# juankim834/RecommendSystemProject

Hardware: AMD Instinct MI355X
Metric: training samples/sec (user-item pairs) at batch 4096; 1/2/4/8 MI355X (higher is better)
Workload: dtype bf16; 1 GPU; c2: MovieLens-1M DSSM + Transformer seq encoder (seq_len 50, d=64); global_batch=4096, per_gpu_batch=4096, seq_len=50, dropout=config, parallelism=dp1, hip_graph=True, ids=uniform, hard_negatives=0, resident_batches=8, deterministic=True

## Files before the change

recommendsystemproject_amd/csrc/attention.hip:

```cpp
#include <type_traits>

#include "attn_rows.h"
#include "common.h"
#include "mfma.h"
#include "rng.h"

namespace rs {
namespace {

__device__ __forceinline__ bool map_bh(int B, int H, int& b, int& h) {
  const int bid = blockIdx.x, xcd = bid & 7, slot = bid >> 3;
  b = (slot / H) * 8 + xcd;
  h = slot % H;
  return b < B;
}

__host__ inline int bh_grid(int B, int H) { return ((B + 7) / 8) * 8 * H; }

template <int HD, bool DROP>
__global__ __launch_bounds__(256) void attn_fwd_kernel(const float* __restrict__ qkv,
                                                       const uint8_t* __restrict__ key_pad,
                                                       float* __restrict__ out,
                                                       float* __restrict__ lse, int B, int L,
                                                       int d, int H, float scale, float pdrop,
// ... 228 lines not shown
    for (int tk = 0; tk < NT; ++tk)
#pragma unroll
      for (int s4 = 0; s4 < 4; ++s4) o = mfma4(sv[tk][s4], Vs[tk * 16 + 4 * q + s4][r], o);
    if (q == 0 && i < L) lse[(int64_t)bh * L + i] = (m + log2f(l)) * kLn2;
#pragma unroll
    for (int e = 0; e < 4; ++e) {
      const float le = __shfl(l, 4 * q + e, 64);
      const int row = tq * 16 + 4 * q + e;
      if (row < L) out[((int64_t)b * L + row) * d + h * 16 + r] = o[e] * (1.f / le);
    }
  }
}

template <int NT, bool DROP>
__global__ __launch_bounds__(256) void attn_bwd_mfma_kernel(
    const float* __restrict__ qkv, const uint8_t* __restrict__ key_pad,
    const float* __restrict__ out, const float* __restrict__ dout, const float* __restrict__ lse,
    float* __restrict__ dqkv, int B, int L, int d, int H, float scale, float pdrop,
    const int64_t* __restrict__ key, int site) {
  constexpr int LP = NT * 16;
  constexpr int TP = 20;
  __shared__ __attribute__((aligned(16))) float Qsm[4][LP][kRowP];
  __shared__ __attribute__((aligned(16))) float Ksm[4][LP][kRowP];
  __shared__ __attribute__((aligned(16))) float Gsm[4][LP][kRowP];
  __shared__ __attribute__((aligned(16))) float Tsm[4][LP * TP];
  const int wave = threadIdx.x >> 6, lane = threadIdx.x & 63;
  const int r = lane & 15, q = lane >> 4;
  const int bh = blockIdx.x * 4 + wave;
  if (bh >= B * H) return;
  const int b = bh / H, h = bh % H;
  const int ld = 3 * d;
  const float* base = qkv + (int64_t)b * L * ld + h * 16;
  const float* gbase = dout + (int64_t)b * L * d + h * 16;
  const float* obase = out + (int64_t)b * L * d + h * 16;
  float(*Qs)[kRowP] = Qsm[wave];
  float(*Ks)[kRowP] = Ksm[wave];
  float(*Gs)[kRowP] = Gsm[wave];
  float* T = Tsm[wave];
  f4 qf[NT], kf[NT], vf[NT], gf[NT];
  float Di[NT], lsei[NT];
#pragma unroll
  for (int t = 0; t < NT; ++t) {
    const int row = t * 16 + r;
    const f4 z = {0.f, 0.f, 0.f, 0.f};
    const bool ok = row < L;
    qf[t] = ok ? ld4(base + (int64_t)row * ld + 4 * q) : z;
    kf[t] = ok ? ld4(base + (int64_t)row * ld + d + 4 * q) : z;
    vf[t] = ok ? ld4(base + (int64_t)row * ld + 2 * d + 4 * q) : z;
    gf[t] = ok ? ld4(gbase + (int64_t)row * d + 4 * q) : z;
    const f4 of = ok ? ld4(obase + (int64_t)row * d + 4 * q) : z;
    *reinterpret_cast<f4*>(&Qs[row][4 * q]) = qf[t];
    *reinterpret_cast<f4*>(&Ks[row][4 * q]) = kf[t];
    *reinterpret_cast<f4*>(&Gs[row][4 * q]) = gf[t];
    Di[t] = quad_sum(gf[t][0] * of[0] + gf[t][1] * of[1] + gf[t][2] * of[2] + gf[t][3] * of[3]);
    lsei[t] = ok ? lse[(int64_t)bh * L + row] * kLog2e : 0.f;
  }
  bool kok[NT][4];
#pragma unroll
  for (int t = 0; t < NT; ++t)
#pragma unroll
    for (int e = 0; e < 4; ++e) {
      const int j = t * 16 + 4 * q + e;
      kok[t][e] = j < L && key_pad[(int64_t)b * L + j] == 0;
    }
  DropKey dk;
  if (DROP) dk = make_key(key, site, pdrop);
  const float scale2 = scale * kLog2e;
  __builtin_amdgcn_wave_barrier();
  float* dbase = dqkv + (int64_t)b * L * ld + h * 16;
  f4 dv_acc[NT], dk_acc[NT];
#pragma unroll
  for (int t = 0; t < NT; ++t) dv_acc[t] = dk_acc[t] = f4{0.f, 0.f, 0.f, 0.f};
#pragma unroll
  for (int tq = 0; tq < NT; ++tq) {
    const int i = tq * 16 + r;
    const uint32_t rowbase = ((uint32_t)bh * (uint32_t)L + (uint32_t)i) * (uint32_t)L;
    f4 ps[NT], ds[NT];
#pragma unroll
    for (int tk = 0; tk < NT; ++tk) {
      f4 sacc = {0.f, 0.f, 0.f, 0.f}, pacc = {0.f, 0.f, 0.f, 0.f};
#pragma unroll
      for (int s4 = 0; s4 < 4; ++s4) {
        sacc = mfma4(kf[tk][s4], qf[tq][s4], sacc);
        pacc = mfma4(vf[tk][s4], gf[tq][s4], pacc);
      }
      float mk[4] = {1.f, 1.f, 1.f, 1.f};
      if (DROP) keep4_32(dk, rowbase + tk * 16 + 4 * q, mk);
#pragma unroll
      for (int e = 0; e < 4; ++e) {
        const float pv = (kok[tk][e] && i < L) ? exp2f(sacc[e] * scale2 - lsei[tq]) : 0.f;
        const float z = DROP ? mk[e] : 1.f;
        ds[tk][e] = pv * (z * pacc[e] - Di[tq]);
        ps[tk][e] = pv * z;
      }
    }
    f4 dq = {0.f, 0.f, 0.f, 0.f};
#pragma unroll
    for (int tk = 0; tk < NT; ++tk)
#pragma unroll
      for (int s4 = 0; s4 < 4; ++s4) dq = mfma4(ds[tk][s4], Ks[tk * 16 + 4 * q + s4][r], dq);
#pragma unroll
    for (int e = 0; e < 4; ++e) {
      const int row = tq * 16 + 4 * q + e;
      if (row < L) dbase[(int64_t)row * ld + r] = dq[e] * scale;
    }
#pragma unroll
    for (int tk = 0; tk < NT; ++tk)
#pragma unroll
      for (int e = 0; e < 4; ++e) T[(tk * 16 + 4 * q + e) * TP + r] = ps[tk][e];
    __builtin_amdgcn_wave_barrier();
#pragma unroll
    for (int tk = 0; tk < NT; ++tk) {
      const f4 a = ld4(&T[(tk * 16 + r) * TP + 4 * q]);
#pragma unroll
      for (int s4 = 0; s4 < 4; ++s4) dv_acc[tk] = mfma4(a[s4], Gs[tq * 16 + 4 * q + s4][r], dv_acc[tk]);
    }
    __builtin_amdgcn_wave_barrier();
#pragma unroll
    for (int tk = 0; tk < NT; ++tk)
#pragma unroll
      for (int e = 0; e < 4; ++e) T[(tk * 16 + 4 * q + e) * TP + r] = ds[tk][e];
    __builtin_amdgcn_wave_barrier();
#pragma unroll
    for (int tk = 0; tk < NT; ++tk) {
      const f4 a = ld4(&T[(tk * 16 + r) * TP + 4 * q]);
#pragma unroll
      for (int s4 = 0; s4 < 4; ++s4) dk_acc[tk] = mfma4(a[s4], Qs[tq * 16 + 4 * q + s4][r], dk_acc[tk]);
    }
    __builtin_amdgcn_wave_barrier();
  }
#pragma unroll
  for (int tk = 0; tk < NT; ++tk)
#pragma unroll
    for (int e = 0; e < 4; ++e) {
      const int row = tk * 16 + 4 * q + e;
      if (row < L) {
        dbase[(int64_t)row * ld + d + r] = dk_acc[tk][e] * scale;
        dbase[(int64_t)row * ld + 2 * d + r] = dv_acc[tk][e];
      }
    }
}


__device__ __forceinline__ shortx4 bf4(const f4& v) {
  typedef __bf16 bf2v __attribute__((ext_vector_type(2)));
  typedef float f2v __attribute__((ext_vector_type(2)));
  const bf2v lo = __builtin_convertvector(f2v{v[0], v[1]}, bf2v);
  const bf2v hi = __builtin_convertvector(f2v{v[2], v[3]}, bf2v);
  return __builtin_bit_cast(shortx4, __builtin_shufflevector(lo, hi, 0, 1, 2, 3));
}
__device__ __forceinline__ f4 mfma16(const shortx4& a, const shortx4& b, const f4& c) {
  return __builtin_amdgcn_mfma_f32_16x16x16bf16_1k(a, b, c, 0, 0, 0);
}
template <int NT, int P>
__device__ __forceinline__ void col_frags(const float* X, int r, int q, shortx4 (&out)[NT]) {
#pragma unroll
  for (int t = 0; t < NT; ++t) {
    f4 v;
#pragma unroll
    for (int j = 0; j < 4; ++j) v[j] = X[(t * 16 + 4 * q + j) * P + r];
    out[t] = bf4(v);
  }
}

__device__ __forceinline__ void stq(float* p, float v) { *p = v; }
__device__ __forceinline__ void stq(__bf16* p, float v) { *p = (__bf16)v; }

template <int NT>
__device__ __forceinline__ uint32_t key_bits(const uint8_t* __restrict__ key_pad, int b, int L,
                                             int lane, int q) {
  const bool valid = lane < L && key_pad[(int64_t)b * L + lane] == 0;
  const uint64_t vm = __ballot(valid);
  uint32_t kb = 0;
#pragma unroll
  for (int t = 0; t < NT; ++t) kb |= (uint32_t)((vm >> (16 * t + 4 * q)) & 0xFu) << (4 * t);
  return kb;
}

__device__ __forceinline__ void attn_keep4(const DropKey& dk, bool leven, uint32_t idx0, float (&mk)[4]) {
  if (leven) {
    keep_pair32(dk, idx0 >> 1, mk[0], mk[1]);
    keep_pair32(dk, (idx0 >> 1) + 1, mk[2], mk[3]);
  } else {
    keep4_32(dk, idx0, mk);
  }
}

__device__ __forceinline__ void attn_keep4b(const DropKey& dk, bool leven, uint32_t idx0, bool (&kp)[4]) {
  if (leven) {
    const uint32_t h0 = pair_hash32(dk, idx0 >> 1), h1 = pair_hash32(dk, (idx0 >> 1) + 1);
    kp[0] = (h0 & 0xffffu) >= dk.thresh;
    kp[1] = (h0 >> 16) >= dk.thresh;
    kp[2] = (h1 & 0xffffu) >= dk.thresh;
    kp[3] = (h1 >> 16) >= dk.thresh;
  } else {
#pragma unroll
    for (int i = 0; i < 4; ++i) {
      const uint32_t x = idx0 + i, hh = pair_hash32(dk, x >> 1);
      kp[i] = ((x & 1) ? (hh >> 16) : (hh & 0xffffu)) >= dk.thresh;
    }
  }
}

template <int NT>
__device__ __forceinline__ void key_bias(uint32_t kbits, f4 (&kbias)[NT]) {
#pragma unroll
  for (int t = 0; t < NT; ++t)
#pragma unroll
    for (int e = 0; e < 4; ++e) kbias[t][e] = ((kbits >> (4 * t + e)) & 1u) ? 0.f : -INFINITY;
}
__device__ __forceinline__ float vmax(float a, float b) { return __builtin_elementwise_maximum(a, b); }

__device__ __forceinline__ shortx4 tr_col(const __bf16* W, int wp, int tk, int lane) {
  const int g = lane >> 4, l16 = lane & 15;
  return tr4(W + (4 * g + (l16 >> 2)) * wp + 16 * tk + 4 * (l16 & 3));
}

template <int TP>
__device__ __forceinline__ f4 tile_rows(float* T, const f4& acc, int r, int q, int lane) {
#pragma unroll
  for (int e = 0; e < 4; ++e) T[(4 * q + e) * TP + r] = acc[e];
  __builtin_amdgcn_wave_barrier();
  const f4 v = ld4(&T[(lane >> 2) * TP + 4 * (lane & 3)]);
  __builtin_amdgcn_wave_barrier();
  return v;
}

template <int NT, bool DROP, bool QB, bool ZB = false>
__global__ __launch_bounds__(256) void attn_fwd_bf16_kernel(
    const void* __restrict__ qkv_, const uint8_t* __restrict__ key_pad, float* __restrict__ out,
    float* __restrict__ lse, int B, int L, int d, int H, float scale, float pdrop,
    const int64_t* __restrict__ key, int site, uint16_t* __restrict__ zbits = nullptr) {
  constexpr int LP = NT * 16;
  __shared__ __attribute__((aligned(16))) float Vsm[4][LP][kRowP];
  const int wave = threadIdx.x >> 6, lane = threadIdx.x & 63;
  const int r = lane & 15, q = lane >> 4;
  const int bh = blockIdx.x * 4 + wave;
  if (bh >= B * H) return;
  const int b = bh / H, h = bh % H;
  const int ld = 3 * d;
  typedef typename std::conditional<QB, __bf16, float>::type QT;
  const QT* base = reinterpret_cast<const QT*>(qkv_) + (int64_t)b * L * ld + h * 16;
  float(*Vs)[kRowP] = Vsm[wave];
  shortx4 qb[NT], kb[NT], vb[NT];
#pragma unroll
  for (int t = 0; t < NT; ++t) {
    const int row = t * 16 + r;
    const f4 z = {0.f, 0.f, 0.f, 0.f};
    qb[t] = bf4(row < L ? ld4(base + (int64_t)row * ld + 4 * q) : z);
    kb[t] = bf4(row < L ? ld4(base + (int64_t)row * ld + d + 4 * q) : z);
    *reinterpret_cast<f4*>(&Vs[row][4 * q]) = row < L ? ld4(base + (int64_t)row * ld + 2 * d + 4 * q) : z;
  }
  const uint32_t kbits = key_bits<NT>(key_pad, b, L, lane, q);
  f4 kbias[NT];
  key_bias<NT>(kbits, kbias);
  DropKey dk;
  if (DROP) dk = make_key(key, site, pdrop);
  const bool leven = (L & 1) == 0;
  const float scale2 = scale * kLog2e;
  __builtin_amdgcn_wave_barrier();
  col_frags<NT, kRowP>(&Vs[0][0], r, q, vb);
  __builtin_amdgcn_wave_barrier();
  float* T = &Vs[0][0];
#pragma unroll
  for (int tq = 0; tq < NT; ++tq) {
    f4 sv[NT];
#pragma unroll
    for (int tk = 0; tk < NT; ++tk) sv[tk] = mfma16(kb[tk], qb[tq], kbias[tk]);
    float m = -INFINITY;
#pragma unroll
    for (int tk = 0; tk < NT; ++tk) m = vmax(vmax(vmax(m, sv[tk][0]), sv[tk][1]), vmax(sv[tk][2], sv[tk][3]));
    m = quad_max(m);
    const float ms = m == -INFINITY ? 0.f : m * scale2;
    float l = 0.f;
    const int i = tq * 16 + r;
    const uint32_t rowbase = ((uint32_t)bh * (uint32_t)L + (uint32_t)i) * (uint32_t)L;
    uint32_t zw = 0;
#pragma unroll
    for (int tk = 0; tk < NT; ++tk) {
      bool kp[4] = {true, true, true, true};
      if (DROP) attn_keep4b(dk, leven, rowbase + tk * 16 + 4 * q, kp);
#pragma unroll
      for (int e = 0; e < 4; ++e) {
        const float pv = __builtin_amdgcn_exp2f(__builtin_fmaf(sv[tk][e], scale2, -ms));
        l += pv;
        sv[tk][e] = kp[e] ? pv : 0.f;
        if (ZB) zw |= kp[e] ? (1u << (4 * tk + e)) : 0u;
      }
    }
    if (ZB) zbits[((int64_t)bh * NT + tq) * 64 + lane] = (uint16_t)zw;
    l = quad_sum(l);
    f4 o = {0.f, 0.f, 0.f, 0.f};
#pragma unroll
    for (int tk = 0; tk < NT; ++tk) o = mfma16(bf4(sv[tk]), vb[tk], o);
    if (q == 0 && i < L) lse[(int64_t)bh * L + i] = (ms + __builtin_amdgcn_logf(l)) * kLn2;
    const float rl = DROP ? __builtin_amdgcn_rcpf(l) * dk.scale : __builtin_amdgcn_rcpf(l);
    f4 on;
#pragma unroll
    for (int e = 0; e < 4; ++e) on[e] = o[e] * __shfl(rl, 4 * q + e, 64);
    const f4 v = tile_rows<kRowP>(T, on, r, q, lane);
    const int row = tq * 16 + (lane >> 2);
    if (row < L) put4(out + ((int64_t)b * L + row) * d + h * 16 + 4 * (lane & 3), v);
  }
}

template <int NT, bool DROP, bool QB, bool ZB = false>
__global__ __launch_bounds__(256, 3) void attn_bwd_bf16_kernel(
    const void* __restrict__ qkv_, const uint8_t* __restrict__ key_pad,
    const float* __restrict__ out, const float* __restrict__ dout, const float* __restrict__ lse,
    void* __restrict__ dqkv_, int B, int L, int d, int H, float scale, float pdrop,
    const int64_t* __restrict__ key, int site, const uint16_t* __restrict__ zbits = nullptr) {
  constexpr int LP = NT * 16;
  constexpr int TP = 24;
  constexpr int WP = LP + 16;
  constexpr int XW = (LP * TP > 16 * TP + 16 * WP) ? LP * TP : 16 * TP + 16 * WP;
  __shared__ __attribute__((aligned(16))) float Xsm[4][XW];
  __shared__ __attribute__((aligned(16))) shortx4 Fsm[4][2][NT][64];
  const int wave = threadIdx.x >> 6, lane = threadIdx.x & 63;
  const int r = lane & 15, q = lane >> 4;
  const int bh = blockIdx.x * 4 + wave;
  if (bh >= B * H) return;
  const int b = bh / H, h = bh % H;
  const int ld = 3 * d;
  typedef typename std::conditional<QB, __bf16, float>::type QT;
  const QT* base = reinterpret_cast<const QT*>(qkv_) + (int64_t)b * L * ld + h * 16;
  const float* gbase = dout + (int64_t)b * L * d + h * 16;
  float* T = Xsm[wave];
  shortx4 qb[NT], kb[NT], vb[NT], gb[NT];
  float lsei[NT];
  shortx4 kc[NT];
  {
    f4 qf[NT], kf[NT], gf[NT];
#pragma unroll
    for (int t = 0; t < NT; ++t) {
      const int row = t * 16 + r;
      const f4 z = {0.f, 0.f, 0.f, 0.f};
      const bool ok = row < L;
      qf[t] = ok ? ld4(base + (int64_t)row * ld + 4 * q) : z;
      kf[t] = ok ? ld4(base + (int64_t)row * ld + d + 4 * q) : z;
      vb[t] = bf4(ok ? ld4(base + (int64_t)row * ld + 2 * d + 4 * q) : z);
      gf[t] = ok ? ld4(gbase + (int64_t)row * d + 4 * q) : z;
      const float ls = ok ? lse[(int64_t)bh * L + row] : 0.f;
      lsei[t] = !ok ? INFINITY : (ls == -INFINITY ? 0.f : ls * kLog2e);
    }
#pragma unroll
    for (int pass = 0; pass < 3; ++pass) {
#pragma unroll
      for (int t = 0; t < NT; ++t)
        *reinterpret_cast<f4*>(&T[(t * 16 + r) * TP + 4 * q]) = pass == 0 ? qf[t] : (pass == 1 ? kf[t] : gf[t]);
      __builtin_amdgcn_wave_barrier();
      if (pass == 1) {
        col_frags<NT, TP>(T, r, q, kc);
      } else {
        shortx4 cf[NT];
        col_frags<NT, TP>(T, r, q, cf);
#pragma unroll
        for (int t = 0; t < NT; ++t) Fsm[wave][pass >> 1][t][lane] = cf[t];
      }
      __builtin_amdgcn_wave_barrier();
    }
#pragma unroll
    for (int t = 0; t < NT; ++t) {
      qb[t] = bf4(qf[t]);
      kb[t] = bf4(kf[t]);
      gb[t] = bf4(gf[t]);
    }
  }
  uint32_t zw[NT];
  if (ZB)
#pragma unroll
    for (int t = 0; t < NT; ++t) zw[t] = zbits[((int64_t)bh * NT + t) * 64 + lane];
  const uint32_t kbits = key_bits<NT>(key_pad, b, L, lane, q);
  f4 kbias[NT];
  key_bias<NT>(kbits, kbias);
  DropKey dk;
  if (DROP) dk = make_key(key, site, pdrop);
  const bool leven = (L & 1) == 0;
  const float scale2 = scale * kLog2e;
  const float zs = DROP ? dk.scale : 1.f;
  QT* dbase = reinterpret_cast<QT*>(dqkv_) + (int64_t)b * L * ld + h * 16;
  __bf16* Wpz = reinterpret_cast<__bf16*>(T + 16 * TP);
  __bf16* Wds = Wpz + 16 * WP;
  f4 dv_acc[NT], dk_acc[NT];
#pragma unroll
  for (int t = 0; t < NT; ++t) dv_acc[t] = dk_acc[t] = f4{0.f, 0.f, 0.f, 0.f};
#pragma unroll
  for (int tq = 0; tq < NT; ++tq) {
    const int i = tq * 16 + r;
    const uint32_t rowbase = ((uint32_t)bh * (uint32_t)L + (uint32_t)i) * (uint32_t)L;
    f4 pvs[NT], dpz[NT];
    float Dp = 0.f;
#pragma unroll
    for (int tk = 0; tk < NT; ++tk) {
      const f4 sacc = mfma16(kb[tk], qb[tq], kbias[tk]);
      const f4 pacc = mfma16(vb[tk], gb[tq], f4{0.f, 0.f, 0.f, 0.f});
      bool kp[4] = {true, true, true, true};
      if (ZB) {
#pragma unroll
        for (int e = 0; e < 4; ++e) kp[e] = (zw[tq] >> (4 * tk + e)) & 1u;
      } else if (DROP) {
        attn_keep4b(dk, leven, rowbase + tk * 16 + 4 * q, kp);
      }
      f4 pz;
#pragma unroll
      for (int e = 0; e < 4; ++e) {
        const float pv = __builtin_amdgcn_exp2f(__builtin_fmaf(sacc[e], scale2, -lsei[tq]));
        pvs[tk][e] = pv;
        dpz[tk][e] = kp[e] ? pacc[e] : 0.f;
        pz[e] = kp[e] ? pv : 0.f;
        Dp = __builtin_fmaf(pv, dpz[tk][e], Dp);
      }
      *reinterpret_cast<shortx4*>(&Wpz[r * WP + 16 * tk + 4 * q]) = bf4(pz);
    }
    const float Di = quad_sum(Dp) * zs;
    f4 dq = {0.f, 0.f, 0.f, 0.f};
#pragma unroll
    for (int tk = 0; tk < NT; ++tk) {
      f4 ds;
#pragma unroll
      for (int e = 0; e < 4; ++e) ds[e] = pvs[tk][e] * __builtin_fmaf(dpz[tk][e], zs, -Di);
      const shortx4 dsb = bf4(ds);
      *reinterpret_cast<shortx4*>(&Wds[r * WP + 16 * tk + 4 * q]) = dsb;
      dq = mfma16(dsb, kc[tk], dq);
    }
    __builtin_amdgcn_wave_barrier();
#pragma unroll
    for (int tk = 0; tk < NT; ++tk) {
      dv_acc[tk] = mfma16(tr_col(Wpz, WP, tk, lane), Fsm[wave][1][tq][lane], dv_acc[tk]);
      dk_acc[tk] = mfma16(tr_col(Wds, WP, tk, lane), Fsm[wave][0][tq][lane], dk_acc[tk]);
    }
    {
      const f4 v = tile_rows<TP>(T, dq * scale, r, q, lane);
      const int row = tq * 16 + (lane >> 2);
      if (row < L) put4(dbase + (int64_t)row * ld + 4 * (lane & 3), v);
    }
    __builtin_amdgcn_wave_barrier();
  }
#pragma unroll
  for (int tk = 0; tk < NT; ++tk) {
    const f4 vk = tile_rows<TP>(T, dk_acc[tk] * scale, r, q, lane);
    const f4 vv = tile_rows<TP>(T, dv_acc[tk] * zs, r, q, lane);
    const int row = tk * 16 + (lane >> 2);
    if (row < L) {
      put4(dbase + (int64_t)row * ld + d + 4 * (lane & 3), vk);
      put4(dbase + (int64_t)row * ld + 2 * d + 4 * (lane & 3), vv);
    }
  }
}

template <int NT>
__device__ __forceinline__ uint64_t key_bits_long(const uint8_t* __restrict__ key_pad, int b,
                                                  int L, int lane, int q) {
  uint64_t kb = 0;
#pragma unroll
  for (int g = 0; g < (NT + 3) / 4; ++g) {
    const int j = 64 * g + lane;
    const uint64_t vm = __ballot(j < L && key_pad[(int64_t)b * L + j] == 0);
#pragma unroll
    for (int tt = 0; tt < 4; ++tt)
      if (4 * g + tt < NT) kb |= ((vm >> (16 * tt + 4 * q)) & 0xFull) << (4 * (4 * g + tt));
  }
  return kb;
}

template <int LP, typename QT>
__device__ __forceinline__ void load_head_image(const QT* __restrict__ base, int ld, int L,
                                                int off, float (*X)[kRowP]) {
  for (int e = threadIdx.x; e < LP * 4; e += 256) {
    const int row = e >> 2, c4 = (e & 3) * 4;
    f4 v = {0.f, 0.f, 0.f, 0.f};
    if (row < L) v = ld4(base + (int64_t)row * ld + off + c4);
    *reinterpret_cast<f4*>(&X[row][c4]) = v;
  }
}

__device__ __forceinline__ void keep_col4(const DropKey& dk, bool leven, uint32_t rb0, uint32_t L,
                                          uint32_t j, int r, float (&mk)[4]) {
  if (leven) {
    const int p = r & 1;
    float mine[2], recv[2];
#pragma unroll
    for (int s = 0; s < 2; ++s) {
      const uint32_t e = 2 * p + s;
      const uint32_t h = pair_hash32(dk, (rb0 + e * L + (j & ~1u)) >> 1);
      const float lo = (h & 0xffffu) >= dk.thresh ? dk.scale : 0.f;
      const float hi = (h >> 16) >= dk.thresh ? dk.scale : 0.f;
      mine[s] = p ? hi : lo;
      recv[s] = __shfl_xor(p ? lo : hi, 1, 64);
    }
#pragma unroll
    for (int e = 0; e < 4; ++e) mk[e] = ((e >> 1) == p) ? mine[e & 1] : recv[e & 1];
  } else {
#pragma unroll
    for (int e = 0; e < 4; ++e) mk[e] = keep_mult32(dk, rb0 + e * L + j);
  }
}

constexpr int kRowPB = 24;
template <int LP, typename QT>
__device__ __forceinline__ void load_head_image16(const QT* __restrict__ base, int ld, int L, int off,
                                                  __bf16 (*X)[kRowPB]) {
  for (int e = threadIdx.x; e < LP * 4; e += 256) {
    const int row = e >> 2, c4 = (e & 3) * 4;
    f4 v = {0.f, 0.f, 0.f, 0.f};
    if (row < L) v = ld4(base + (int64_t)row * ld + off + c4);
    *reinterpret_cast<shortx4*>(&X[row][c4]) = bf4(v);
  }
}
__device__ __forceinline__ shortx4 row_frag16(const __bf16 (*X)[kRowPB], int row, int q) {
  return *reinterpret_cast<const shortx4*>(&X[row][4 * q]);
}
__device__ __forceinline__ shortx4 col_frag16(const __bf16 (*X)[kRowPB], int t0, int r, int q) {
  shortx4 o;
#pragma unroll
  for (int j = 0; j < 4; ++j) o[j] = __builtin_bit_cast(short, X[t0 + 4 * q + j][r]);
  return o;
}

#ifndef RS_LONG_FWD_MINW
#define RS_LONG_FWD_MINW 3
#endif
template <int NT, bool DROP, bool QB>
__global__ __launch_bounds__(256, RS_LONG_FWD_MINW) void attn_fwd_long_bf16_kernel(
    const void* __restrict__ qkv_, const uint8_t* __restrict__ key_pad, float* __restrict__ out,
    float* __restrict__ lse, int B, int L, int d, int H, float scale, float pdrop,
    const int64_t* __restrict__ key, int site) {
  constexpr int LP = NT * 16;
  __shared__ __attribute__((aligned(16))) __bf16 Qs[LP][kRowPB];
  __shared__ __attribute__((aligned(16))) __bf16 Ks[LP][kRowPB];
  __shared__ __attribute__((aligned(16))) __bf16 Vs[LP][kRowPB];
  __shared__ __attribute__((aligned(16))) float Tsm[4][16 * kRowP];
  __shared__ __attribute__((aligned(16))) float Kb[LP];
  int b, h;
  if (!map_bh(B, H, b, h)) return;
  const int bh = b * H + h;
  const int wave = threadIdx.x >> 6, lane = threadIdx.x & 63;
  const int r = lane & 15, q = lane >> 4;
  const int ld = 3 * d;
  typedef typename std::conditional<QB, __bf16, float>::type QT;
  const QT* base = reinterpret_cast<const QT*>(qkv_) + (int64_t)b * L * ld + h * 16;
  load_head_image16<LP>(base, ld, L, 0, Qs);
  load_head_image16<LP>(base, ld, L, d, Ks);
  load_head_image16<LP>(base, ld, L, 2 * d, Vs);
  for (int j = threadIdx.x; j < LP; j += 256) Kb[j] = (j < L && key_pad[(int64_t)b * L + j] == 0) ? 0.f : -INFINITY;
  DropKey dk;
  if (DROP) dk = make_key(key, site, pdrop);
  const bool leven = (L & 1) == 0;
  const float scale2 = scale * kLog2e;
  __syncthreads();
  shortx4 kb[NT];
#pragma unroll
  for (int t = 0; t < NT; ++t) kb[t] = row_frag16(Ks, t * 16 + r, q);
  float* T = Tsm[wave];
  constexpr int NTF = 4 * (NT / 4), NR = NT - NTF;
  for (int tq = wave; tq < NTF; tq += 4) {
    const int i = tq * 16 + r;
    const f4 z = {0.f, 0.f, 0.f, 0.f};
    const shortx4 qb = row_frag16(Qs, i, q);
    constexpr int CH = 4;
    float m = -INFINITY, ms = 0.f, l = 0.f;
    f4 o = z;
    const uint32_t rowbase = ((uint32_t)bh * (uint32_t)L + (uint32_t)i) * (uint32_t)L;
#pragma unroll
    for (int c0 = 0; c0 < NT; c0 += CH) {
      f4 sv[CH];
      float cm = -INFINITY;
#pragma unroll
      for (int u = 0; u < CH; ++u) {
        const int tk = c0 + u;
        if (tk >= NT) break;
        sv[u] = mfma16(kb[tk], qb, ld4(&Kb[tk * 16 + 4 * q]));
        cm = vmax(vmax(vmax(cm, sv[u][0]), sv[u][1]), vmax(sv[u][2], sv[u][3]));
      }
      cm = quad_max(cm);
      const float mn = vmax(m, cm);
      const float msn = mn == -INFINITY ? 0.f : mn * scale2;
      if (c0 > 0) {
        const float al = m == -INFINITY ? 0.f : __builtin_amdgcn_exp2f(ms - msn);
        l *= al;
#pragma unroll
        for (int e = 0; e < 4; ++e) o[e] *= __shfl(al, 4 * q + e, 64);
      }
      m = mn;
      ms = msn;
#pragma unroll
      for (int u = 0; u < CH; ++u) {
        const int tk = c0 + u;
        if (tk >= NT) break;
        bool kp[4] = {true, true, true, true};
        if (DROP) attn_keep4b(dk, leven, rowbase + tk * 16 + 4 * q, kp);
#pragma unroll
        for (int e = 0; e < 4; ++e) {
          const float pv = __builtin_amdgcn_exp2f(__builtin_fmaf(sv[u][e], scale2, -ms));
          l += pv;
// ... 151 lines not shown
    L2s[i] = li;
    Kv[i] = kv;
  }
  DropKey dk;
  if (DROP) dk = make_key(key, site, pdrop);
  const bool leven = (L & 1) == 0;
  const float scale2 = scale * kLog2e;
  const f4 z = {0.f, 0.f, 0.f, 0.f};
  float* T = reinterpret_cast<float*>(Tbs[wave]);
  __bf16* Tb = Tbs[wave];
  QT* dbase = reinterpret_cast<QT*>(dqkv_) + (int64_t)b * L * ld + h * 16;
  __syncthreads();

  shortx4 kr[NW], vr[NW], kc[NW];
  float kval[NW];
  f4 dk_acc[NW], dv_acc[NW], dq_acc[NT];
#pragma unroll
  for (int u = 0; u < NW; ++u) {
    const int tk = u < NW0 ? wave + 4 * u : NTF + (u - NW0);
    kr[u] = row_frag16(Ks, tk * 16 + r, q);
    vr[u] = row_frag16(Vs, tk * 16 + r, q);
    kc[u] = col_frag16(Ks, tk * 16, r, q);
    kval[u] = Kv[tk * 16 + r];
    dk_acc[u] = dv_acc[u] = z;
  }
#pragma unroll
  for (int tq = 0; tq < NT; ++tq) {
    const shortx4 qr = row_frag16(Qs, tq * 16 + r, q);
    const shortx4 gr = row_frag16(Gs, tq * 16 + r, q);
    const shortx4 qc[1] = {col_frag16(Qs, tq * 16, r, q)};
    const shortx4 gc[1] = {col_frag16(Gs, tq * 16, r, q)};
    const f4 l2 = ld4(&L2s[tq * 16 + 4 * q]);
    const f4 Dq = ld4(&Ds[tq * 16 + 4 * q]);
    dq_acc[tq] = z;
#pragma unroll
    for (int u = 0; u < NW; ++u) {
      const int tk = u < NW0 ? wave + 4 * u : NTF + (u - NW0);
      if (u >= NW0 && (tq & 3) != wave) continue;
      const f4 sacc = mfma16(qr, kr[u], z);
      const f4 pacc = mfma16(gr, vr[u], z);
      float mk[4] = {1.f, 1.f, 1.f, 1.f};
      if (DROP)
        keep_col4(dk, leven, ((uint32_t)bh * (uint32_t)L + (uint32_t)(tq * 16 + 4 * q)) * (uint32_t)L,
                  (uint32_t)L, (uint32_t)(tk * 16 + r), r, mk);
      f4 pz, ds;
#pragma unroll
      for (int e = 0; e < 4; ++e) {
        float pv = __builtin_amdgcn_exp2f(__builtin_fmaf(sacc[e], scale2, -l2[e]));
        pv = kval[u] != 0.f ? pv : 0.f;
        pz[e] = pv * mk[e];
        ds[e] = pv * __builtin_fmaf(mk[e], pacc[e], -Dq[e]);
      }
      dv_acc[u] = mfma16(bf4(pz), gc[0], dv_acc[u]);
      const shortx4 dsb = bf4(ds);
      dk_acc[u] = mfma16(dsb, qc[0], dk_acc[u]);
      const bf16x4 dh = __builtin_bit_cast(bf16x4, dsb);
#pragma unroll
      for (int e = 0; e < 4; ++e) Tb[u * 16 * TPB + (4 * q + e) * TPB + r] = dh[e];
    }
    __builtin_amdgcn_wave_barrier();
#pragma unroll
    for (int u = 0; u < NW; ++u) {
      if (u >= NW0 && (tq & 3) != wave) continue;
      const shortx4 dst = *reinterpret_cast<const shortx4*>(&Tb[u * 16 * TPB + r * TPB + 4 * q]);
      dq_acc[tq] = mfma16(dst, kc[u], dq_acc[tq]);
    }
    __builtin_amdgcn_wave_barrier();
  }
#pragma unroll
  for (int u = 0; u < NW0; ++u) {
    const int tk = wave + 4 * u;
    const f4 vk = tile_rows<TP>(T, dk_acc[u] * scale, r, q, lane);
    const f4 vv = tile_rows<TP>(T, dv_acc[u], r, q, lane);
    const int row = tk * 16 + (lane >> 2);
    if (row < L) {
      put4(dbase + (int64_t)row * ld + d + 4 * (lane & 3), vk);
      put4(dbase + (int64_t)row * ld + 2 * d + 4 * (lane & 3), vv);
    }
  }
  __syncthreads();
  float* accq = reinterpret_cast<float*>(&img[0][0][0]);
  f4* accs = reinterpret_cast<f4*>(accq + LP * 16);
  for (int w = 0; w < 4; ++w) {
    if (wave == w) {
#pragma unroll
      for (int tq = 0; tq < NT; ++tq)
#pragma unroll
        for (int e = 0; e < 4; ++e) {
          float* pp = accq + (tq * 16 + 4 * q + e) * 16 + r;
          *pp = (w == 0 ? 0.f : *pp) + dq_acc[tq][e];
        }
#pragma unroll
      for (int x = 0; x < NR; ++x) {
        f4* pk = accs + (x * 2 + 0) * 64 + lane;
        f4* pv = accs + (x * 2 + 1) * 64 + lane;
        *pk = (w == 0 ? z : *pk) + dk_acc[NW0 + x];
        *pv = (w == 0 ? z : *pv) + dv_acc[NW0 + x];
      }
    }
    __syncthreads();
  }
  if constexpr (NR > 0) {
    if (wave < NR) {
      const int x = wave;
      const f4 vk = tile_rows<TP>(T, accs[(x * 2 + 0) * 64 + lane] * scale, r, q, lane);
      const f4 vv = tile_rows<TP>(T, accs[(x * 2 + 1) * 64 + lane], r, q, lane);
      const int row = (NTF + x) * 16 + (lane >> 2);
      if (row < L) {
        put4(dbase + (int64_t)row * ld + d + 4 * (lane & 3), vk);
        put4(dbase + (int64_t)row * ld + 2 * d + 4 * (lane & 3), vv);
      }
    }
  }
  for (int e = threadIdx.x; e < LP * 4; e += 256) {
    const int row = e >> 2, c4 = (e & 3) * 4;
    if (row >= L) continue;
    put4(dbase + (int64_t)row * ld + c4, ld4(accq + row * 16 + c4) * scale);
  }
}

int threads_for(int L) {
  int t = ((L + 63) / 64) * 64;
  return t > 256 ? 256 : t;
}

size_t valu_lds(int L, int hd, int bwd) {
  return (size_t)(bwd ? 4 * L * hd + 3 * L : 2 * L * hd + L) * sizeof(float);
}

int attn_plan(const char* fn, int B, int L, int d, int H, float p, int flags, int bwd, rs_attn_plan_t* out) {
  RS_CHECK_ARG(B >= 0 && L >= 1 && H >= 1 && d % H == 0, "%s: bad shape", fn);
  RS_CHECK_ARG(p >= 0.f && p < 1.f, "%s: bad dropout p=%f", fn, p);
  const int hd = d / H;
  RS_CHECK_ARG(head_dim_ok(hd), "%s: head_dim %d unsupported", fn, hd);
  const bool bf = (flags & RS_GEMM_BF16) != 0;
  const bool mfma_ok = hd == 16 && (int64_t)B * H * L * L < ((int64_t)1 << 32) && !getenv_flag("RSYS_ATTN_VALU");
  rs_attn_plan_t pl = {};
  pl.route = mfma_ok && L <= 64              ? (bf ? RS_ATTN_WAVE_BF16 : RS_ATTN_WAVE_F32)
             : mfma_ok && bf && L <= 256     ? RS_ATTN_LONG_BF16
                                             : RS_ATTN_VALU;
  pl.nt = pl.route == RS_ATTN_VALU ? 0 : (L + 15) / 16;
  pl.qkv_bf16 = pl.route == RS_ATTN_WAVE_BF16 || pl.route == RS_ATTN_LONG_BF16;
  pl.zbits_words = pl.route == RS_ATTN_WAVE_BF16 && p > 0.f ? (int64_t)B * H * pl.nt * 64 : 0;
  pl.rows_ok = attn_rows_ok(L, hd);
  if (out) *out = pl;
  RS_CHECK_ARG(B == 0 || pl.route != RS_ATTN_VALU || valu_lds(L, hd, bwd) <= 64 * 1024,
               "%s: L=%d hd=%d exceeds LDS", fn, L, hd);
  RS_CHECK_ARG(B == 0 || !(flags & RS_ATTN_QKV_BF16) || pl.qkv_bf16,
               "%s: bf16 qkv storage needs the bf16 MFMA path (RS_GEMM_BF16, head_dim 16, L <= 256, "
               "B*H*L*L < 2^32, RSYS_ATTN_VALU off)", fn);
  return 0;
}

int attn_check(const char* fn, bool pointers, const void* qkv, const void* io, int B, int L, int d, int H,
               float p, const int64_t* key, int flags, int bwd, rs_attn_plan_t* plan) {
  RS_CHECK_ARG(pointers, "%s: null pointer", fn);
  RS_RET_IF(attn_plan(fn, B, L, d, H, p, flags, bwd, plan));
  RS_CHECK_ARG(p == 0.f || key, "%s: bad dropout p=%f", fn, p);
  RS_CHECK_ARG(B == 0 || (d % 4 == 0 && aligned16(qkv) && aligned16(io)), "%s: needs 16-byte aligned rows", fn);
  return 0;
}

}
}

using namespace rs;

extern "C" int rs_attn_plan(int B, int L, int d, int H, float p, int flags, int bwd, rs_attn_plan_t* out) {
  return attn_plan("rs_attn_plan", B, L, d, H, p, flags, bwd, out);
}

extern "C" int rs_attn_fwd(const float* qkv, const uint8_t* key_pad, float* out, float* lse,
                           int B, int L, int d, int H, float scale, float p, const int64_t* key,
                           int site, int flags, void* stream, uint16_t* zbits) {
  rs_attn_plan_t plan;
  RS_RET_IF(attn_check("rs_attn_fwd", qkv && key_pad && out && lse, qkv, out, B, L, d, H, p, key, flags, 0,
                       &plan));
  if (B == 0) return 0;
  hipStream_t st = as_stream(stream);
  const dim3 g4(cdiv((int64_t)B * H, 4)), gbh(bh_grid(B, H));
  const bool drop = p > 0.f, qb = (flags & RS_ATTN_QKV_BF16) != 0;
  const int zmode = drop + (drop && zbits);
  switch (plan.route) {
    case RS_ATTN_WAVE_F32:
      for_int<1, 4>(plan.nt, [&](auto nt) { for_bool(drop, [&](auto dr) {
        attn_fwd_mfma_kernel<nt.value, dr.value>
            <<<g4, 256, 0, st>>>(qkv, key_pad, out, lse, B, L, d, H, scale, p, key, site);
      }); });
      break;
    case RS_ATTN_WAVE_BF16:
      for_int<1, 4>(plan.nt, [&](auto nt) { for_bool(qb, [&](auto q) { for_int<0, 2>(zmode, [&](auto dm) {
        attn_fwd_bf16_kernel<nt.value, dm.value != 0, q.value, dm.value == 2>
            <<<g4, 256, 0, st>>>(qkv, key_pad, out, lse, B, L, d, H, scale, p, key, site,
                                 dm.value == 2 ? zbits : nullptr);
      }); }); });
      break;
    case RS_ATTN_LONG_BF16:
      for_int<5, 16>(plan.nt, [&](auto nt) { for_bool(qb, [&](auto q) { for_bool(drop, [&](auto dr) {
        attn_fwd_long_bf16_kernel<nt.value, dr.value, q.value>
            <<<gbh, 256, 0, st>>>(qkv, key_pad, out, lse, B, L, d, H, scale, p, key, site);
      }); }); });
      break;
    default:
      for_int<0, 3>(__builtin_ctz(d / H) - 3, [&](auto i) { for_bool(drop, [&](auto dr) {
        attn_fwd_kernel<(8 << i.value), dr.value><<<gbh, threads_for(L), valu_lds(L, d / H, 0), st>>>(
            qkv, key_pad, out, lse, B, L, d, H, scale, p, key, site);
      }); });
  }
  RS_CHECK_LAUNCH("rs_attn_fwd");
  return 0;
}

extern "C" int rs_attn_bwd(const float* qkv, const uint8_t* key_pad, const float* out,
                           const float* dout, const float* lse, float* dqkv, int B, int L, int d,
                           int H, float scale, float p, const int64_t* key, int site, int flags,
                           void* stream, const uint16_t* zbits) {
  rs_attn_plan_t plan;
  RS_RET_IF(attn_check("rs_attn_bwd", qkv && key_pad && out && dout && lse && dqkv, qkv, dout, B, L, d, H, p, key,
                       flags, 1, &plan));
  if (B == 0) return 0;
  RS_CHECK_ARG(plan.route == RS_ATTN_VALU || aligned16(out), "rs_attn_bwd: needs 16-byte aligned rows");
  hipStream_t st = as_stream(stream);
  const dim3 g4(cdiv((int64_t)B * H, 4)), gbh(bh_grid(B, H));
  const bool drop = p > 0.f, qb = (flags & RS_ATTN_QKV_BF16) != 0;
  const int zmode = drop + (drop && zbits);
  switch (plan.route) {
    case RS_ATTN_WAVE_F32:
      for_int<1, 4>(plan.nt, [&](auto nt) { for_bool(drop, [&](auto dr) {
        attn_bwd_mfma_kernel<nt.value, dr.value>
            <<<g4, 256, 0, st>>>(qkv, key_pad, out, dout, lse, dqkv, B, L, d, H, scale, p, key, site);
      }); });
      break;
    case RS_ATTN_WAVE_BF16:
      for_int<1, 4>(plan.nt, [&](auto nt) { for_bool(qb, [&](auto q) { for_int<0, 2>(zmode, [&](auto dm) {
        attn_bwd_bf16_kernel<nt.value, dm.value != 0, q.value, dm.value == 2><<<g4, 256, 0, st>>>(
            qkv, key_pad, out, dout, lse, dqkv, B, L, d, H, scale, p, key, site, dm.value == 2 ? zbits : nullptr);
      }); }); });
      break;
    case RS_ATTN_LONG_BF16:
      for_int<5, 16>(plan.nt, [&](auto nt) { for_bool(qb, [&](auto q) { for_bool(drop, [&](auto dr) {
        attn_bwd_long1_bf16_kernel<nt.value, dr.value, q.value>
            <<<gbh, 256, 0, st>>>(qkv, key_pad, out, dout, lse, dqkv, B, L, d, H, scale, p, key, site);
      }); }); });
      break;
    default:
      for_int<0, 3>(__builtin_ctz(d / H) - 3, [&](auto i) { for_bool(drop, [&](auto dr) {
        attn_bwd_kernel<(8 << i.value), dr.value><<<gbh, threads_for(L), valu_lds(L, d / H, 1), st>>>(
            qkv, key_pad, out, dout, lse, dqkv, B, L, d, H, scale, p, key, site);
      }); });
  }
  RS_CHECK_LAUNCH("rs_attn_bwd");
  return 0;
}
```

Baseline: 3.749 million samples/s.

## Skip fully padded key tiles and zero-gradient query tiles in bf16 attention

```diff
diff --git a/recommendsystemproject_amd/csrc/attention.hip b/recommendsystemproject_amd/csrc/attention.hip
--- a/recommendsystemproject_amd/csrc/attention.hip
+++ b/recommendsystemproject_amd/csrc/attention.hip
@@ -404,10 +404,20 @@
 __device__ __forceinline__ f4 mfma16(const shortx4& a, const shortx4& b, const f4& c) {
   return __builtin_amdgcn_mfma_f32_16x16x16bf16_1k(a, b, c, 0, 0, 0);
 }
+template <bool SK = true>
+__device__ __forceinline__ bool tile_on(uint32_t mask, int t) {
+  if (!SK) return true;
+  uint32_t m = __builtin_amdgcn_readfirstlane(mask);
+  asm volatile("" : "+s"(m));
+  return (m >> t) & 1u;
+}
+
 template <int NT, int P>
-__device__ __forceinline__ void col_frags(const float* X, int r, int q, shortx4 (&out)[NT]) {
+__device__ __forceinline__ void col_frags(const float* X, int r, int q, shortx4 (&out)[NT], uint32_t mask = ~0u) {
 #pragma unroll
   for (int t = 0; t < NT; ++t) {
+    out[t] = shortx4{0, 0, 0, 0};
+    if (mask != ~0u && !tile_on(mask, t)) continue;
     f4 v;
 #pragma unroll
     for (int j = 0; j < 4; ++j) v[j] = X[(t * 16 + 4 * q + j) * P + r];
@@ -420,14 +430,22 @@
 
 template <int NT>
 __device__ __forceinline__ uint32_t key_bits(const uint8_t* __restrict__ key_pad, int b, int L,
-                                             int lane, int q) {
+                                             int lane, int q, int skip, uint32_t& live, uint32_t& part) {
   const bool valid = lane < L && key_pad[(int64_t)b * L + lane] == 0;
   const uint64_t vm = __ballot(valid);
-  uint32_t kb = 0;
-#pragma unroll
-  for (int t = 0; t < NT; ++t) kb |= (uint32_t)((vm >> (16 * t + 4 * q)) & 0xFu) << (4 * t);
+  uint32_t kb = 0, lv = 0, full = 0;
+#pragma unroll
+  for (int t = 0; t < NT; ++t) {
+    const uint32_t tile = (uint32_t)(vm >> (16 * t)) & 0xFFFFu;
+    kb |= ((tile >> (4 * q)) & 0xFu) << (4 * t);
+    lv |= tile ? 1u << t : 0u;
+    full |= tile == 0xFFFFu ? 1u << t : 0u;
+  }
+  live = __builtin_amdgcn_readfirstlane(skip ? lv : (1u << NT) - 1u);
+  part = live & ~__builtin_amdgcn_readfirstlane(full);
   return kb;
 }
+
 
 __device__ __forceinline__ void attn_keep4(const DropKey& dk, bool leven, uint32_t idx0, float (&mk)[4]) {
   if (leven) {
@@ -454,12 +472,10 @@
   }
 }
 
-template <int NT>
-__device__ __forceinline__ void key_bias(uint32_t kbits, f4 (&kbias)[NT]) {
-#pragma unroll
-  for (int t = 0; t < NT; ++t)
-#pragma unroll
-    for (int e = 0; e < 4; ++e) kbias[t][e] = ((kbits >> (4 * t + e)) & 1u) ? 0.f : -INFINITY;
+__device__ __forceinline__ f4 mask_scores(f4 s, uint32_t kbits, int t) {
+#pragma unroll
+  for (int e = 0; e < 4; ++e) s[e] = ((kbits >> (4 * t + e)) & 1u) ? s[e] : -INFINITY;
+  return s;
 }
 __device__ __forceinline__ float vmax(float a, float b) { return __builtin_elementwise_maximum(a, b); }
 
@@ -482,7 +498,7 @@
 __global__ __launch_bounds__(256) void attn_fwd_bf16_kernel(
     const void* __restrict__ qkv_, const uint8_t* __restrict__ key_pad, float* __restrict__ out,
     float* __restrict__ lse, int B, int L, int d, int H, float scale, float pdrop,
-    const int64_t* __restrict__ key, int site, uint16_t* __restrict__ zbits = nullptr) {
+    const int64_t* __restrict__ key, int site, int skip, uint16_t* __restrict__ zbits = nullptr) {
   constexpr int LP = NT * 16;
   __shared__ __attribute__((aligned(16))) float Vsm[4][LP][kRowP];
   const int wave = threadIdx.x >> 6, lane = threadIdx.x & 63;
@@ -494,42 +510,50 @@
   typedef typename std::conditional<QB, __bf16, float>::type QT;
   const QT* base = reinterpret_cast<const QT*>(qkv_) + (int64_t)b * L * ld + h * 16;
   float(*Vs)[kRowP] = Vsm[wave];
+  uint32_t live, part;
+  const uint32_t kbits = key_bits<NT>(key_pad, b, L, lane, q, skip, live, part);
   shortx4 qb[NT], kb[NT], vb[NT];
 #pragma unroll
   for (int t = 0; t < NT; ++t) {
     const int row = t * 16 + r;
     const f4 z = {0.f, 0.f, 0.f, 0.f};
     qb[t] = bf4(row < L ? ld4(base + (int64_t)row * ld + 4 * q) : z);
+    kb[t] = shortx4{0, 0, 0, 0};
+    if (!tile_on(live, t)) continue;
     kb[t] = bf4(row < L ? ld4(base + (int64_t)row * ld + d + 4 * q) : z);
     *reinterpret_cast<f4*>(&Vs[row][4 * q]) = row < L ? ld4(base + (int64_t)row * ld + 2 * d + 4 * q) : z;
   }
-  const uint32_t kbits = key_bits<NT>(key_pad, b, L, lane, q);
-  f4 kbias[NT];
-  key_bias<NT>(kbits, kbias);
   DropKey dk;
   if (DROP) dk = make_key(key, site, pdrop);
   const bool leven = (L & 1) == 0;
   const float scale2 = scale * kLog2e;
   __builtin_amdgcn_wave_barrier();
-  col_frags<NT, kRowP>(&Vs[0][0], r, q, vb);
+  col_frags<NT, kRowP>(&Vs[0][0], r, q, vb, live);
   __builtin_amdgcn_wave_barrier();
   float* T = &Vs[0][0];
 #pragma unroll
   for (int tq = 0; tq < NT; ++tq) {
     f4 sv[NT];
 #pragma unroll
-    for (int tk = 0; tk < NT; ++tk) sv[tk] = mfma16(kb[tk], qb[tq], kbias[tk]);
+    for (int tk = 0; tk < NT; ++tk)
+      if (tile_on(live, tk)) {
+        sv[tk] = mfma16(kb[tk], qb[tq], f4{0.f, 0.f, 0.f, 0.f});
+        if (tile_on(part, tk)) sv[tk] = mask_scores(sv[tk], kbits, tk);
+      }
     float m = -INFINITY;
 #pragma unroll
-    for (int tk = 0; tk < NT; ++tk) m = vmax(vmax(vmax(m, sv[tk][0]), sv[tk][1]), vmax(sv[tk][2], sv[tk][3]));
+    for (int tk = 0; tk < NT; ++tk)
+      if (tile_on(live, tk)) m = vmax(vmax(vmax(m, sv[tk][0]), sv[tk][1]), vmax(sv[tk][2], sv[tk][3]));
     m = quad_max(m);
     const float ms = m == -INFINITY ? 0.f : m * scale2;
     float l = 0.f;
     const int i = tq * 16 + r;
     const uint32_t rowbase = ((uint32_t)bh * (uint32_t)L + (uint32_t)i) * (uint32_t)L;
     uint32_t zw = 0;
+    f4 o = {0.f, 0.f, 0.f, 0.f};
 #pragma unroll
     for (int tk = 0; tk < NT; ++tk) {
+      if (!tile_on(live, tk)) continue;
       bool kp[4] = {true, true, true, true};
       if (DROP) attn_keep4b(dk, leven, rowbase + tk * 16 + 4 * q, kp);
 #pragma unroll
@@ -539,12 +563,10 @@
         sv[tk][e] = kp[e] ? pv : 0.f;
         if (ZB) zw |= kp[e] ? (1u << (4 * tk + e)) : 0u;
       }
+      o = mfma16(bf4(sv[tk]), vb[tk], o);
     }
     if (ZB) zbits[((int64_t)bh * NT + tq) * 64 + lane] = (uint16_t)zw;
     l = quad_sum(l);
-    f4 o = {0.f, 0.f, 0.f, 0.f};
-#pragma unroll
-    for (int tk = 0; tk < NT; ++tk) o = mfma16(bf4(sv[tk]), vb[tk], o);
     if (q == 0 && i < L) lse[(int64_t)bh * L + i] = (ms + __builtin_amdgcn_logf(l)) * kLn2;
     const float rl = DROP ? __builtin_amdgcn_rcpf(l) * dk.scale : __builtin_amdgcn_rcpf(l);
     f4 on;
@@ -561,7 +583,7 @@
     const void* __restrict__ qkv_, const uint8_t* __restrict__ key_pad,
     const float* __restrict__ out, const float* __restrict__ dout, const float* __restrict__ lse,
     void* __restrict__ dqkv_, int B, int L, int d, int H, float scale, float pdrop,
-    const int64_t* __restrict__ key, int site, const uint16_t* __restrict__ zbits = nullptr) {
+    const int64_t* __restrict__ key, int site, int skip, const uint16_t* __restrict__ zbits = nullptr) {
   constexpr int LP = NT * 16;
   constexpr int TP = 24;
   constexpr int WP = LP + 16;
@@ -578,6 +600,9 @@
   const QT* base = reinterpret_cast<const QT*>(qkv_) + (int64_t)b * L * ld + h * 16;
   const float* gbase = dout + (int64_t)b * L * d + h * 16;
   float* T = Xsm[wave];
+  constexpr bool SK = DROP && NT > 2;
+  uint32_t klive_all, kpart, qlive = 0;
+  const uint32_t kbits = key_bits<NT>(key_pad, b, L, lane, q, SK ? skip : 0, klive_all, kpart);
   shortx4 qb[NT], kb[NT], vb[NT], gb[NT];
   float lsei[NT];
   shortx4 kc[NT];
@@ -596,18 +621,27 @@
       lsei[t] = !ok ? INFINITY : (ls == -INFINITY ? 0.f : ls * kLog2e);
     }
 #pragma unroll
+    for (int t = 0; t < NT; ++t) {
+      const bool nz = gf[t][0] != 0.f || gf[t][1] != 0.f || gf[t][2] != 0.f || gf[t][3] != 0.f;
+      qlive |= __ballot(nz) ? 1u << t : 0u;
+    }
+    qlive = __builtin_amdgcn_readfirstlane(skip ? qlive : (1u << NT) - 1u);
+#pragma unroll
     for (int pass = 0; pass < 3; ++pass) {
+      const uint32_t on = pass == 1 ? klive_all : qlive;
 #pragma unroll
       for (int t = 0; t < NT; ++t)
-        *reinterpret_cast<f4*>(&T[(t * 16 + r) * TP + 4 * q]) = pass == 0 ? qf[t] : (pass == 1 ? kf[t] : gf[t]);
+        if (tile_on<SK>(on, t))
+          *reinterpret_cast<f4*>(&T[(t * 16 + r) * TP + 4 * q]) = pass == 0 ? qf[t] : (pass == 1 ? kf[t] : gf[t]);
       __builtin_amdgcn_wave_barrier();
       if (pass == 1) {
-        col_frags<NT, TP>(T, r, q, kc);
+        col_frags<NT, TP>(T, r, q, kc, SK ? on : ~0u);
       } else {
         shortx4 cf[NT];
-        col_frags<NT, TP>(T, r, q, cf);
-#pragma unroll
-        for (int t = 0; t < NT; ++t) Fsm[wave][pass >> 1][t][lane] = cf[t];
+        col_frags<NT, TP>(T, r, q, cf, SK ? on : ~0u);
+#pragma unroll
+        for (int t = 0; t < NT; ++t)
+          if (tile_on<SK>(on, t)) Fsm[wave][pass >> 1][t][lane] = cf[t];
       }
       __builtin_amdgcn_wave_barrier();
     }
@@ -622,9 +656,6 @@
   if (ZB)
 #pragma unroll
     for (int t = 0; t < NT; ++t) zw[t] = zbits[((int64_t)bh * NT + t) * 64 + lane];
-  const uint32_t kbits = key_bits<NT>(key_pad, b, L, lane, q);
-  f4 kbias[NT];
-  key_bias<NT>(kbits, kbias);
   DropKey dk;
   if (DROP) dk = make_key(key, site, pdrop);
   const bool leven = (L & 1) == 0;
@@ -638,13 +669,17 @@
   for (int t = 0; t < NT; ++t) dv_acc[t] = dk_acc[t] = f4{0.f, 0.f, 0.f, 0.f};
 #pragma unroll
   for (int tq = 0; tq < NT; ++tq) {
+    const uint32_t klive = tile_on<SK>(qlive, tq) ? klive_all : 0u;
     const int i = tq * 16 + r;
     const uint32_t rowbase = ((uint32_t)bh * (uint32_t)L + (uint32_t)i) * (uint32_t)L;
     f4 pvs[NT], dpz[NT];
+    const shortx4 qcol = Fsm[wave][0][tq][lane], gcol = Fsm[wave][1][tq][lane];
     float Dp = 0.f;
 #pragma unroll
     for (int tk = 0; tk < NT; ++tk) {
-      const f4 sacc = mfma16(kb[tk], qb[tq], kbias[tk]);
+      if (!tile_on<SK>(klive, tk)) continue;
+      f4 sacc = mfma16(kb[tk], qb[tq], f4{0.f, 0.f, 0.f, 0.f});
+      if (tile_on(kpart, tk)) sacc = mask_scores(sacc, kbits, tk);
       const f4 pacc = mfma16(vb[tk], gb[tq], f4{0.f, 0.f, 0.f, 0.f});
       bool kp[4] = {true, true, true, true};
       if (ZB) {
@@ -668,6 +703,7 @@
     f4 dq = {0.f, 0.f, 0.f, 0.f};
 #pragma unroll
     for (int tk = 0; tk < NT; ++tk) {
+      if (!tile_on<SK>(klive, tk)) continue;
       f4 ds;
 #pragma unroll
       for (int e = 0; e < 4; ++e) ds[e] = pvs[tk][e] * __builtin_fmaf(dpz[tk][e], zs, -Di);
@@ -678,8 +714,9 @@
     __builtin_amdgcn_wave_barrier();
 #pragma unroll
     for (int tk = 0; tk < NT; ++tk) {
-      dv_acc[tk] = mfma16(tr_col(Wpz, WP, tk, lane), Fsm[wave][1][tq][lane], dv_acc[tk]);
-      dk_acc[tk] = mfma16(tr_col(Wds, WP, tk, lane), Fsm[wave][0][tq][lane], dk_acc[tk]);
+      if (!tile_on<SK>(klive, tk)) continue;
+      dv_acc[tk] = mfma16(tr_col(Wpz, WP, tk, lane), gcol, dv_acc[tk]);
+      dk_acc[tk] = mfma16(tr_col(Wds, WP, tk, lane), qcol, dk_acc[tk]);
     }
     {
       const f4 v = tile_rows<TP>(T, dq * scale, r, q, lane);
@@ -690,8 +727,11 @@
   }
 #pragma unroll
   for (int tk = 0; tk < NT; ++tk) {
-    const f4 vk = tile_rows<TP>(T, dk_acc[tk] * scale, r, q, lane);
-    const f4 vv = tile_rows<TP>(T, dv_acc[tk] * zs, r, q, lane);
+    f4 vk = {0.f, 0.f, 0.f, 0.f}, vv = vk;
+    if (tile_on<SK>(klive_all, tk)) {
+      vk = tile_rows<TP>(T, dk_acc[tk] * scale, r, q, lane);
+      vv = tile_rows<TP>(T, dv_acc[tk] * zs, r, q, lane);
+    }
     const int row = tk * 16 + (lane >> 2);
     if (row < L) {
       put4(dbase + (int64_t)row * ld + d + 4 * (lane & 3), vk);
@@ -1149,6 +1189,11 @@
   return 0;
 }
 
+int skip_tiles() {
+  const char* v = getenv("RSYS_ATTN_SKIP_TILES");
+  return !(v && v[0] == '0' && v[1] == 0);
+}
+
 int attn_check(const char* fn, bool pointers, const void* qkv, const void* io, int B, int L, int d, int H,
                float p, const int64_t* key, int flags, int bwd, rs_attn_plan_t* plan) {
   RS_CHECK_ARG(pointers, "%s: null pointer", fn);
@@ -1188,7 +1233,7 @@
     case RS_ATTN_WAVE_BF16:
       for_int<1, 4>(plan.nt, [&](auto nt) { for_bool(qb, [&](auto q) { for_int<0, 2>(zmode, [&](auto dm) {
         attn_fwd_bf16_kernel<nt.value, dm.value != 0, q.value, dm.value == 2>
-            <<<g4, 256, 0, st>>>(qkv, key_pad, out, lse, B, L, d, H, scale, p, key, site,
+            <<<g4, 256, 0, st>>>(qkv, key_pad, out, lse, B, L, d, H, scale, p, key, site, skip_tiles(),
                                  dm.value == 2 ? zbits : nullptr);
       }); }); });
       break;
@@ -1231,7 +1276,8 @@
     case RS_ATTN_WAVE_BF16:
       for_int<1, 4>(plan.nt, [&](auto nt) { for_bool(qb, [&](auto q) { for_int<0, 2>(zmode, [&](auto dm) {
         attn_bwd_bf16_kernel<nt.value, dm.value != 0, q.value, dm.value == 2><<<g4, 256, 0, st>>>(
-            qkv, key_pad, out, dout, lse, dqkv, B, L, d, H, scale, p, key, site, dm.value == 2 ? zbits : nullptr);
+            qkv, key_pad, out, dout, lse, dqkv, B, L, d, H, scale, p, key, site, skip_tiles(),
+            dm.value == 2 ? zbits : nullptr);
       }); }); });
       break;
     case RS_ATTN_LONG_BF16:
```

Result: faster. 3.787 million samples/s (median of 5 runs) (+1.0%).
